# DSXiangLi/ChineseNER

Hardware: NVIDIA H100
Metric: sentences/sec bert_bilstm_crf MSRA L=128 (higher is better)
Workload: dtype bf16

## Files before the change

chinesener_b200/_lib.py:

```python
import ctypes
import os

import torch

_HERE = os.path.dirname(os.path.abspath(__file__))
LIB_PATH = os.path.join(_HERE, "libner_b200.so")

_c = ctypes
_vp, _i = _c.c_void_p, _c.c_int

SIGNATURES = {
    "ner_strerror": (_c.c_char_p, [_i]),
    "ner_abi_version": (_i, []),
    "ner_build_info": (_c.c_char_p, []),
    "ner_crf_viterbi": (_i, [_vp, _vp, _vp, _vp, _vp, _i, _i, _i, _vp]),
    "ner_crf_viterbi_plan": (_i, [_i, _i, _i, _i, _i]),
    "ner_crf_loglik_fwd": (_i, [_vp, _vp, _vp, _vp, _vp, _vp, _vp, _i, _i, _i, _i, _vp]),
    "ner_crf_loglik_bwd": (_i, [_vp, _vp, _vp, _vp, _vp, _vp, _vp, _c.c_float, _vp, _vp, _i, _i, _i, _vp]),
    "ner_gemm_bf16": (_i, [_vp, _vp, _vp, _vp, _vp, _i, _i, _i, _i, _i, _vp]),
    "ner_pack_weight_bf16": (_i, [_vp, _vp, _i, _i, _vp]),
    "ner_cast_bf16": (_i, [_vp, _vp, _c.c_size_t, _vp]),
    "ner_dense_small_n": (_i, [_vp, _i, _vp, _vp, _vp, _i, _i, _i, _vp, _vp]),
    "ner_seq_pack_plan": (_i, [_vp, _vp, _vp, _i, _i, _vp]),
    "ner_bert_embed_ln": (_i, [_vp] * 9 + [_i] * 6 + [_c.c_float, _vp, _i, _vp]),
    "ner_layernorm": (_i, [_vp, _i] + [_vp] * 5 + [_i, _i, _c.c_float, _vp]),
    "ner_layernorm_dropout": (_i, [_vp, _i] + [_vp] * 5 + [_i, _i, _c.c_float, _c.c_float, _c.c_uint64, _vp]),
    "ner_bert_attention": (_i, [_vp, _vp, _vp, _i, _i, _i, _i, _c.c_float, _c.c_float, _vp, _i, _c.c_float, _c.c_uint64, _vp]),
    "ner_bilstm_recurrence": (_i, [_vp] * 5 + [_i, _i, _i, _i, _c.c_float, _vp, _vp, _vp, _vp, _c.c_float, _c.c_uint64, _vp]),
    "ner_bilstm_recurrence_bwd": (_i, [_vp] * 7 + [_i, _i, _i, _i, _c.c_float, _c.c_uint64, _vp]),
    "ner_bigru_recurrence": (_i, [_vp] * 5 + [_i, _i, _i, _i, _i] + [_vp] * 4 + [_c.c_float, _c.c_uint64, _vp]),
    "ner_bigru_recurrence_bwd": (_i, [_vp] * 7 + [_i, _i, _i, _i, _c.c_float, _c.c_uint64, _vp]),
    "ner_transpose_cast_bf16": (_i, [_vp, _vp, _i, _i, _i, _i, _vp]),
    "ner_colsum_add": (_i, [_vp, _vp, _i, _i, _i, _c.c_float, _vp]),
    "ner_dense_small_n_bwd": (_i, [_vp] * 6 + [_i, _i, _i, _vp]),
    "ner_dropout": (_i, [_vp, _vp, _c.c_size_t, _c.c_float, _c.c_uint64, _vp]),
    "ner_relu_bwd_f32": (_i, [_vp, _vp, _vp, _c.c_size_t, _vp]),
    "ner_relu_f32": (_i, [_vp, _vp, _c.c_size_t, _vp]),
    "ner_reduce_max_time": (_i, [_vp, _vp, _i, _i, _i, _vp]),
    "ner_reduce_max_time_bwd": (_i, [_vp, _vp, _vp, _vp, _i, _i, _i, _c.c_float, _vp]),
    "ner_softmax_xent": (_i, [_vp, _vp, _vp, _vp, _i, _i, _c.c_float, _vp]),
    "ner_attention_f32_bwd": (_i, [_vp, _i, _vp, _i, _vp, _i, _vp, _vp, _vp, _vp, _c.c_float, _vp, _i, _vp, _i, _vp, _i, _vp, _i,
                                   _vp, _vp, _i, _i, _i, _i, _vp]),
    "ner_dropout_bf16": (_i, [_vp, _vp, _c.c_size_t, _c.c_float, _c.c_uint64, _vp]),
    "ner_sumsq_add": (_i, [_vp, _c.c_size_t, _vp, _vp, _vp]),
    "ner_sumsq_scratch_floats": (_c.c_size_t, []),
    "ner_token_xent": (_i, [_vp] * 6 + [_c.c_float, _vp, _i, _i, _i, _vp]),
    "ner_token_xent_scratch_floats": (_c.c_size_t, []),
    "ner_token_dice": (_i, [_vp] * 6 + [_c.c_float] * 3 + [_vp, _i, _i, _i, _vp]),
    "ner_mrc_pairs": (_i, [_vp] * 6 + [_i] * 6 + [_vp] * 7),
    "ner_mrc_merge": (_i, [_vp] * 3 + [_i] * 6 + [_vp, _vp]),
    "ner_mrc_span_targets": (_i, [_vp, _vp, _i, _i, _vp, _vp, _vp, _vp]),
    "ner_mrc_span_match_fwd_workspace_bytes": (_c.c_size_t, [_i, _i]),
    "ner_mrc_span_match_fwd": (_i, [_vp, _i] + [_vp] * 5 + [_i] * 3 + [_c.c_float, _c.c_uint64] + [_vp] * 3
                               + [_c.c_size_t, _vp]),
    "ner_mrc_span_match_bwd_workspace_bytes": (_c.c_size_t, [_i, _i]),
    "ner_mrc_span_match_bwd": (_i, [_vp, _i] + [_vp] * 5 + [_i] * 3 + [_c.c_float, _c.c_float, _c.c_uint64] + [_vp] * 5
                               + [_c.c_size_t, _vp]),
    "ner_mrc_span_decode_workspace_bytes": (_c.c_size_t, [_i, _i]),
    "ner_mrc_span_decode": (_i, [_vp] * 3 + [_i] + [_vp] * 5 + [_i] * 8 + [_vp] * 5 + [_c.c_size_t, _vp]),
    "ner_gp_targets": (_i, [_vp] * 3 + [_i] * 3 + [_vp, _vp]),
    "ner_gp_rope": (_i, [_vp, _i, _vp] + [_i] * 3 + [_vp] * 3),
    "ner_gp_rope_bwd": (_i, [_vp, _vp] + [_i] * 3 + [_vp, _i, _vp]),
    "ner_gp_loss_workspace_bytes": (_c.c_size_t, [_i] * 3),
    "ner_gp_loss_fwd": (_i, [_vp] * 5 + [_i] * 3 + [_vp] * 3 + [_c.c_size_t, _vp]),
    "ner_gp_loss_bwd": (_i, [_vp] * 5 + [_i] * 3 + [_c.c_float, _vp, _vp]),
    "ner_gp_decode_workspace_bytes": (_c.c_size_t, [_i] * 3),
    "ner_gp_decode": (_i, [_vp] * 5 + [_i] * 7 + [_vp] * 5 + [_c.c_size_t, _vp]),
    "ner_window_plan": (_i, [_vp] * 3 + [_i] * 5 + [_vp] * 6),
    "ner_layernorm_bwd": (_i, [_vp, _i] + [_vp] * 7 + [_i, _i, _c.c_float, _vp]),
    "ner_layernorm_dropout_bwd": (_i, [_vp, _i] + [_vp] * 7 + [_i, _i, _c.c_float, _c.c_float, _c.c_uint64, _vp]),
    "ner_layernorm_dropout_bwd_bias": (_i, [_vp, _i] + [_vp] * 8 + [_i, _i, _c.c_float, _c.c_float, _c.c_uint64, _vp]),
    "ner_transpose_bf16": (_i, [_vp, _vp, _i, _i, _i, _vp]),
    "ner_colsum_bf16_add": (_i, [_vp, _vp, _i, _i, _vp]),
    "ner_gelu_bf16": (_i, [_vp, _vp, _c.c_size_t, _i, _vp]),
    "ner_gelu_f32": (_i, [_vp, _vp, _c.c_size_t, _i, _vp]),
    "ner_gelu_bwd_bf16": (_i, [_vp, _vp, _vp, _c.c_size_t, _i, _vp]),
    "ner_gelu_bwd_bias_bf16": (_i, [_vp, _vp, _vp, _vp, _i, _i, _i, _vp]),
    "ner_bert_embed_bwd": (_i, [_vp] * 6 + [_i] * 5 + [_vp]),
    "ner_bert_attention_bwd": (_i, [_vp] * 5 + [_i] * 4 + [_c.c_float, _c.c_float, _c.c_float, _c.c_uint64, _vp]),
    "ner_bert_attention_bwd_packed": (_i, [_vp] * 5 + [_i] * 4 + [_c.c_float, _c.c_float, _c.c_uint64, _vp]),
    "ner_gather_rows": (_i, [_vp, _vp, _vp, _i, _i, _vp]),
# ... 148 lines not shown
```

chinesener_b200/csrc/bilstm.cu:

```cuda
#include <cooperative_groups.h>
#include <stdlib.h>

#include "common.cuh"
#include "dsmem.cuh"

namespace cg = cooperative_groups;

namespace {

__device__ __forceinline__ float sigmoidf_(float x) { return __fdividef(1.f, 1.f + __expf(-x)); }

template <int ACT>
__device__ __forceinline__ float actf(float x) {
  if (ACT == 1) return fmaxf(x, 0.f);
  return 1.f - __fdividef(2.f, 1.f + __expf(2.f * x));
}

template <int R, int ACT, int H4REG>
__global__ void __launch_bounds__(H4REG > 0 ? 256 : 512, 1) bilstm_rec_kernel(const float* __restrict__ xproj, const float* __restrict__ wh_fw,
                                  const float* __restrict__ wh_bw, const int32_t* __restrict__ seq_len,
                                  float* __restrict__ out, int B, int L, int H, int C, float forget_bias,
                                  const int32_t* __restrict__ cu_seqlens, float* __restrict__ gates_out,
                                  float* __restrict__ cstate_out, float* __restrict__ hstate_out, float keep_prob,
                                  uint32_t seed_lo, uint32_t seed_hi) {
  cg::cluster_group cluster = cg::this_cluster();
  const int rank = (int)cluster.block_rank();
  const int HU = H / C;
  const int NC = 4 * HU;
  const int H4 = H / 4;
  const int ngroups = (B + R - 1) / R;
  const int cid = blockIdx.x / C;
  const int dir = cid / ngroups;
  const int b0 = (cid % ngroups) * R;
  const int tid = threadIdx.x;

  extern __shared__ __align__(16) float smem[];
  constexpr bool WREG = H4REG > 0;
  float4* Ws4 = reinterpret_cast<float4*>(smem);
  float* hbuf = smem + (WREG ? 0 : (size_t)H * NC);
  int* s_len = reinterpret_cast<int*>(hbuf + 2 * R * H);
  uint64_t* hbar = reinterpret_cast<uint64_t*>(s_len + 8);

  const float* wh = dir == 0 ? wh_fw : wh_bw;
  float4 wreg[WREG ? H4REG : 1];
  if constexpr (WREG) {
    if (tid < NC) {
      const int g0 = tid & 3, u0 = tid >> 2;
      const size_t gc = (size_t)g0 * H + rank * HU + u0;
#pragma unroll
      for (int k4 = 0; k4 < H4REG; ++k4) {
        wreg[k4].x = wh[(size_t)(4 * k4 + 0) * 4 * H + gc];
        wreg[k4].y = wh[(size_t)(4 * k4 + 1) * 4 * H + gc];
        wreg[k4].z = wh[(size_t)(4 * k4 + 2) * 4 * H + gc];
        wreg[k4].w = wh[(size_t)(4 * k4 + 3) * 4 * H + gc];
      }
    }
  } else {
    for (int idx = tid; idx < H4 * NC; idx += blockDim.x) {
      const int k4 = idx / NC, col = idx - k4 * NC;
      const int g = col & 3, u = col >> 2;
      const size_t gc = (size_t)g * H + rank * HU + u;
      float4 w;
      w.x = wh[(size_t)(4 * k4 + 0) * 4 * H + gc];
      w.y = wh[(size_t)(4 * k4 + 1) * 4 * H + gc];
      w.z = wh[(size_t)(4 * k4 + 2) * 4 * H + gc];
      w.w = wh[(size_t)(4 * k4 + 3) * 4 * H + gc];
      Ws4[idx] = w;
    }
  }
  for (int idx = tid; idx < 2 * R * H; idx += blockDim.x) hbuf[idx] = 0.f;
  if (tid < R) s_len[tid] = (b0 + tid < B) ? min(max(seq_len[b0 + tid], 0), L) : 0;
  if (tid == 0) {
    mbar_init_(&hbar[0], 1);
    mbar_init_(&hbar[1], 1);
    asm volatile("fence.mbarrier_init.release.cluster;" ::: "memory");
  }
  __syncthreads();
  int maxlen = 0;
#pragma unroll
  for (int r = 0; r < R; ++r) maxlen = max(maxlen, s_len[r]);
  cluster.sync();

  const bool col_ok = tid < NC;
  const int g = tid & 3, u = tid >> 2;
  const int ug = rank * HU + u;
  const size_t xcol = (size_t)dir * 4 * H + (size_t)g * H + ug;
  constexpr int RC = (R + 3) / 4;
  float c_state[RC];
#pragma unroll
  for (int rr = 0; rr < RC; ++rr) c_state[rr] = 0.f;

  size_t xrow0[R];
#pragma unroll
  for (int r = 0; r < R; ++r)
    xrow0[r] = (b0 + r < B) ? (cu_seqlens ? (size_t)cu_seqlens[b0 + r] : (size_t)(b0 + r) * L) : 0;
  float xp[R];
#pragma unroll
  for (int r = 0; r < R; ++r) {
    xp[r] = 0.f;
    const int len = s_len[r];
    if (col_ok && 0 < len) {
      const int pos = dir == 0 ? 0 : len - 1;
      xp[r] = xproj[(xrow0[r] + pos) * 8 * H + xcol];
    }
  }
  const uint32_t thr = nerdev::keep_threshold(keep_prob);
  const float inv_keep = 1.f / keep_prob;

  const uint32_t h_bytes = (uint32_t)(R * H * 4);
  for (int s = 0; s < maxlen; ++s) {
    const float* hcur = hbuf + (s & 1) * R * H;
    float* hnxt = hbuf + ((s + 1) & 1) * R * H;
    if (C > 1) {
      if (tid == 0) mbar_arrive_expect_tx_(&hbar[(s + 1) & 1], h_bytes);
      if (s > 0) mbar_wait_(&hbar[s & 1], (uint32_t)((s - 1) >> 1) & 1u);
    }
    nerdev::f32x2 pa[R], pb[R];
#pragma unroll
    for (int r = 0; r < R; ++r) {
      pa[r] = nerdev::pk2(xp[r], 0.f);
      pb[r] = nerdev::pk2(0.f, 0.f);
    }
    if (col_ok) {
#pragma unroll
      for (int r = 0; r < R; ++r) {
        const int len = s_len[r];
        xp[r] = 0.f;
        if (s + 1 < len) {
          const int pos = dir == 0 ? s + 1 : len - 2 - s;
          xp[r] = xproj[(xrow0[r] + pos) * 8 * H + xcol];
        }
      }
      const float4* hc4 = reinterpret_cast<const float4*>(hcur);
      if constexpr (WREG) {
#pragma unroll
        for (int k4 = 0; k4 < H4REG; ++k4) {
          const float4 w = wreg[k4];
#pragma unroll
          for (int r = 0; r < R; ++r) {
            const float4 hv = hc4[r * H4 + k4];
            pa[r] = nerdev::fma2(nerdev::pk2(w.x, w.y), nerdev::pk2(hv.x, hv.y), pa[r]);
            pb[r] = nerdev::fma2(nerdev::pk2(w.z, w.w), nerdev::pk2(hv.z, hv.w), pb[r]);
          }
        }
      } else {
#pragma unroll 4
        for (int k4 = 0; k4 < H4; ++k4) {
          const float4 w = Ws4[k4 * NC + tid];
#pragma unroll
          for (int r = 0; r < R; ++r) {
            const float4 hv = hc4[r * H4 + k4];
            pa[r] = nerdev::fma2(nerdev::pk2(w.x, w.y), nerdev::pk2(hv.x, hv.y), pa[r]);
            pb[r] = nerdev::fma2(nerdev::pk2(w.z, w.w), nerdev::pk2(hv.z, hv.w), pb[r]);
          }
        }
      }
    }
    float zi[RC], zj[RC], zf[RC], zo[RC];
#pragma unroll
    for (int rr = 0; rr < RC; ++rr) zi[rr] = zj[rr] = zf[rr] = zo[rr] = 0.f;
    const int qb = (tid & 31) & ~3;
#pragma unroll
    for (int r = 0; r < R; ++r) {
      float z0, z1, z2, z3;
      nerdev::upk2(pa[r], z0, z1);
      nerdev::upk2(pb[r], z2, z3);
      const float z = (z0 + z1) + (z2 + z3);
      const float a0 = __shfl_sync(0xffffffffu, z, qb + 0);
      const float a1 = __shfl_sync(0xffffffffu, z, qb + 1);
      const float a2 = __shfl_sync(0xffffffffu, z, qb + 2);
      const float a3 = __shfl_sync(0xffffffffu, z, qb + 3);
      if (g == (r & 3)) {
        zi[r >> 2] = a0;
        zj[r >> 2] = a1;
        zf[r >> 2] = a2;
        zo[r >> 2] = a3;
      }
    }
#pragma unroll
    for (int rr = 0; rr < RC; ++rr) {
      const int r = g + 4 * rr;
      const bool cell_ok = col_ok && r < R;
      float i_s = 0.f, j_a = 0.f, f_s = 0.f, o_s = 0.f, h_out = 0.f, h_state = 0.f;
      const int len = cell_ok ? s_len[r] : 0;
      const int b = b0 + r;
      const bool live = cell_ok && s < len;
      const int pos = dir == 0 ? s : len - 1 - s;
      if (live) {
        i_s = sigmoidf_(zi[rr]);
        j_a = actf<ACT>(zj[rr]);
        f_s = sigmoidf_(zf[rr] + forget_bias);
        o_s = sigmoidf_(zo[rr]);
        c_state[rr] = f_s * c_state[rr] + i_s * j_a;
        const float h_raw = o_s * actf<ACT>(c_state[rr]);
        h_out = h_raw;
        h_state = h_raw;
        if (keep_prob < 1.f) {
          const uint32_t e = (uint32_t)(((size_t)b * L + pos) * 2 * H + (size_t)dir * H + ug);
          h_out = nerdev::hash3(seed_lo, seed_hi, e) < thr ? h_raw * inv_keep : 0.f;
          h_state = nerdev::hash3(seed_lo ^ 0x5bd1e995u, seed_hi, e) < thr ? h_raw * inv_keep : 0.f;
        }
      }
      if (cell_ok) {
        if (C > 1) {
          const uint32_t la = nerdev::smem_u32(hnxt + r * H + ug), lb = nerdev::smem_u32(&hbar[(s + 1) & 1]);
          for (int dst = 0; dst < C; ++dst) st_async_f32(mapa_u32(la, (uint32_t)dst), h_state, mapa_u32(lb, (uint32_t)dst));
        } else {
          hnxt[r * H + ug] = h_state;
        }
      }
      if (live) {
        out[((size_t)b * L + pos) * 2 * H + (size_t)dir * H + ug] = h_out;
        if (hstate_out != nullptr) hstate_out[((size_t)b * L + pos) * 2 * H + (size_t)dir * H + ug] = h_state;
        if (gates_out != nullptr) {
          const size_t gi = ((size_t)b * L + pos) * 8 * H + (size_t)dir * 4 * H;
          gates_out[gi + 0 * H + ug] = i_s;
          gates_out[gi + 1 * H + ug] = j_a;
          gates_out[gi + 2 * H + ug] = f_s;
          gates_out[gi + 3 * H + ug] = o_s;
          cstate_out[((size_t)b * L + pos) * 2 * H + (size_t)dir * H + ug] = c_state[rr];
        }
      } else if (cell_ok && b < B) {
        out[((size_t)b * L + s) * 2 * H + (size_t)dir * H + ug] = 0.f;
      }
    }
    if (C == 1) __syncthreads();
  }
  if (C > 1) cluster.sync();

  for (int idx = tid; idx < R * HU; idx += blockDim.x) {
    const int r = idx / HU, uu = idx - r * HU;
    const int b = b0 + r;
    if (b < B)
      for (int s = maxlen; s < L; ++s) out[((size_t)b * L + s) * 2 * H + (size_t)dir * H + rank * HU + uu] = 0.f;
  }
}

int pick_cluster(int H) {
  for (int C = 1; C <= 8; C *= 2) {
    if (H % C != 0) continue;
    const size_t bytes = (size_t)H * 4 * (H / C) * 4;
    if (bytes <= 190 * 1024 && 4 * (H / C) <= 512) return C;
  }
  return 0;
}

template <int R, int ACT, int H4REG>
int launch_rec(const float* xproj, const float* wh_fw, const float* wh_bw, const int32_t* seq_len, float* out, int B,
               int L, int H, int C, float forget_bias, const int32_t* cu_seqlens, float* gates_out, float* cstate_out,
               float* hstate_out, float keep_prob, uint64_t seed, cudaStream_t st) {
  const int HU = H / C, NC = 4 * HU;
  const size_t smem = ((H4REG > 0 ? 0 : (size_t)H * NC) + 2 * R * H + 32) * 4;
  auto kern = bilstm_rec_kernel<R, ACT, H4REG>;
  cudaError_t e = cudaFuncSetAttribute(kern, cudaFuncAttributeMaxDynamicSharedMemorySize, (int)smem);
  if (e != cudaSuccess) return NER_ERR_CUDA_BASE - (int)e;
  const int ngroups = (B + R - 1) / R;
  cudaLaunchConfig_t cfg{};
  cfg.gridDim = dim3((unsigned)(2 * ngroups * C));
  cfg.blockDim = dim3((unsigned)((NC + 31) / 32 * 32));
  cfg.dynamicSmemBytes = smem;
  cfg.stream = st;
  cudaLaunchAttribute attr[1];
  attr[0].id = cudaLaunchAttributeClusterDimension;
  attr[0].val.clusterDim.x = (unsigned)C;
  attr[0].val.clusterDim.y = 1;
  attr[0].val.clusterDim.z = 1;
  cfg.attrs = attr;
  cfg.numAttrs = 1;
  e = cudaLaunchKernelEx(&cfg, kern, xproj, wh_fw, wh_bw, seq_len, out, B, L, H, C, forget_bias, cu_seqlens, gates_out,
                         cstate_out, hstate_out, keep_prob, (uint32_t)seed, (uint32_t)(seed >> 32));
  if (e != cudaSuccess) return NER_ERR_CUDA_BASE - (int)e;
  return ner_launch_status();
}

}

extern "C" int ner_bilstm_recurrence(const float* xproj, const float* wh_fw, const float* wh_bw,
                                     const int32_t* seq_len, float* out, int B, int L, int H, int activation,
                                     float forget_bias, const int32_t* cu_seqlens, float* gates_out,
                                     float* cstate_out, float* hstate_out, float keep_prob, uint64_t seed,
                                     ner_stream_t stream) {
  if (B < 0 || L < 1 || H < 1) return NER_ERR_INVALID_ARG;
  if (B == 0) return NER_OK;
  if (!xproj || !wh_fw || !wh_bw || !seq_len || !out) return NER_ERR_INVALID_ARG;
  if ((gates_out == nullptr) != (cstate_out == nullptr)) return NER_ERR_INVALID_ARG;
  if (!(keep_prob > 0.f) || keep_prob > 1.f) return NER_ERR_INVALID_ARG;
  if (activation != 0 && activation != 1) return NER_ERR_INVALID_ARG;
  if (H % 4 != 0) return NER_ERR_UNSUPPORTED;
  const int C = pick_cluster(H);
  if (C == 0) return NER_ERR_UNSUPPORTED;
  cudaStream_t st = static_cast<cudaStream_t>(stream);
  int R = 1;
  if ((long)2 * B * C > ner_num_sms()) R = 2;
  if ((long)2 * ((B + 1) / 2) * C > 2 * ner_num_sms()) R = 4;
  if (H == 128 && (long)2 * ((B + 3) / 4) * C > ner_num_sms()) R = 8;
  if (const char* e = getenv("NER_BILSTM_ROWS")) {
    const int v = atoi(e);
    if (v == 1 || v == 2 || v == 4 || (v == 8 && H == 128)) R = v;
  }
#define GO(RR, HR)                                                                                          \
  return activation == 1 ? launch_rec<RR, 1, HR>(xproj, wh_fw, wh_bw, seq_len, out, B, L, H, C, forget_bias, cu_seqlens, gates_out, cstate_out, hstate_out, keep_prob, seed, st) \
                         : launch_rec<RR, 0, HR>(xproj, wh_fw, wh_bw, seq_len, out, B, L, H, C, forget_bias, cu_seqlens, gates_out, cstate_out, hstate_out, keep_prob, seed, st)
  if (H == 128 && 4 * (H / C) <= 256) {
    if (R == 8) GO(8, 32);
    if (R == 4) GO(4, 32);
    if (R == 2) GO(2, 32);
    GO(1, 32);
  }
  if (R >= 4) GO(4, 0);
  if (R == 2) GO(2, 0);
  GO(1, 0);
#undef GO
}
```

chinesener_b200/csrc/predict_step.cu:

```cuda
#include "common.cuh"

namespace {
inline size_t al256(size_t x) { return (x + 255) & ~(size_t)255; }
}

extern "C" size_t ner_bert_bilstm_crf_predict_workspace_bytes(const ner_bert_config* cfg, int B, int L, int rows,
                                                              int lstm_hidden, int num_tags) {
  if (!cfg || B < 0 || L < 1 || rows < 0) return 0;
  const size_t H = (size_t)cfg->hidden_size, R = (size_t)rows, Hl = (size_t)lstm_hidden;
  return al256((size_t)(B + 1) * 4)
         + al256((size_t)B * L * 4)
         + al256(R * H * 4) + al256(R * H * 2)
         + al256(R * 8 * Hl * 4)
         + al256((size_t)B * L * 2 * Hl * 4)
         + al256((size_t)B * L * num_tags * 4)
         + ner_bert_encoder_workspace_bytes(cfg, rows);
}

extern "C" int ner_bert_bilstm_crf_predict(const ner_bert_config* cfg, const float* word_emb, const float* type_emb,
                                           const float* pos_emb, const float* emb_ln_gamma, const float* emb_ln_beta,
                                           const ner_bert_layer_weights* layers, const void* lstm_wx_bf16,
                                           const float* lstm_bias, const float* lstm_wh_fw, const float* lstm_wh_bw,
                                           int lstm_hidden, int lstm_activation, const float* logits_w,
                                           const float* logits_b, const float* trans, int num_tags, const int32_t* ids,
                                           const int32_t* mask, const int32_t* seg, const int32_t* seq_len, int B, int L,
                                           int n_packed, int32_t* pred_ids, void* workspace, size_t workspace_bytes,
                                           ner_stream_t stream) {
  if (!cfg || !layers || !lstm_wx_bf16 || !lstm_bias || !lstm_wh_fw || !lstm_wh_bw || !logits_w || !logits_b || !trans ||
      !ids || !mask || !seq_len || !pred_ids || !workspace)
    return NER_ERR_INVALID_ARG;
  if (B < 0 || L < 1 || n_packed < 0 || n_packed > B * L) return NER_ERR_INVALID_ARG;
  if (B == 0) return NER_OK;
  const int H = cfg->hidden_size, Hl = lstm_hidden, K = num_tags;
  if (H % 8 != 0) return NER_ERR_UNSUPPORTED;
  if (workspace_bytes < ner_bert_bilstm_crf_predict_workspace_bytes(cfg, B, L, n_packed, Hl, K)) return NER_ERR_WORKSPACE;
  cudaStream_t st = static_cast<cudaStream_t>(stream);
  uint8_t* p = static_cast<uint8_t*>(workspace);
  int32_t* cu = reinterpret_cast<int32_t*>(p);       p += al256((size_t)(B + 1) * 4);
  int32_t* tok_src = reinterpret_cast<int32_t*>(p);  p += al256((size_t)B * L * 4);
  float* x32 = reinterpret_cast<float*>(p);          p += al256((size_t)n_packed * H * 4);
  void* x16 = p;                                     p += al256((size_t)n_packed * H * 2);
  float* xproj = reinterpret_cast<float*>(p);        p += al256((size_t)n_packed * 8 * Hl * 4);
  float* lstm_out = reinterpret_cast<float*>(p);     p += al256((size_t)B * L * 2 * Hl * 4);
  float* logits = reinterpret_cast<float*>(p);       p += al256((size_t)B * L * K * 4);
  void* enc_ws = p;
  const size_t enc_bytes = ner_bert_encoder_workspace_bytes(cfg, n_packed);

  int rc = ner_seq_pack_plan(mask, cu, tok_src, B, L, stream);
  if (rc != NER_OK) return rc;
  if (n_packed == 0) {
    if (cudaMemsetAsync(pred_ids, 0, (size_t)B * L * 4, st) != cudaSuccess) return NER_ERR_CUDA_BASE - (int)cudaGetLastError();
    return NER_OK;
  }
  rc = ner_bert_encoder_fwd(cfg, word_emb, type_emb, pos_emb, emb_ln_gamma, emb_ln_beta, layers, ids, mask, seg, B, L, cu,
                            tok_src, n_packed, x32, x16, enc_ws, enc_bytes, stream);
  if (rc != NER_OK) return rc;
  rc = ner_gemm_bf16(x16, lstm_wx_bf16, lstm_bias, nullptr, xproj, n_packed, 8 * Hl, H, NER_EPI_F32, cfg->gemm_tile, stream);
  if (rc != NER_OK) return rc;
  rc = ner_bilstm_recurrence(xproj, lstm_wh_fw, lstm_wh_bw, seq_len, lstm_out, B, L, Hl, lstm_activation, 1.0f, cu, nullptr,
                             nullptr, nullptr, 1.0f, 0, stream);
  if (rc != NER_OK) return rc;
  rc = ner_dense_small_n(lstm_out, 0, logits_w, logits_b, logits, B * L, 2 * Hl, K, nullptr, stream);
  if (rc != NER_OK) return rc;
  return ner_crf_viterbi(logits, seq_len, trans, pred_ids, nullptr, B, L, K, stream);
}
```

chinesener_b200/fastpath.py:

```python
import ctypes

import torch

from . import _lib, bert as _bert, ops
from .tools import layer as _layer

_ws = {}


def _workspace(nbytes, device):
    key = (device.index, _lib.stream())
    ws = _ws.get(key)
    if ws is None or ws.numel() < nbytes:
        ws = _ws[key] = torch.empty((nbytes,), dtype=torch.uint8, device=device)
    return ws


def bert_bilstm_crf_predict(est, dev):
    store, params = est.store, est.params
    mask = dev['mask']
    total = getattr(mask, "total_tokens", None)
    if total is None or not _layer.PACK_SEQUENCES or _bert.PER_KERNEL or params.get('bert_precision', _layer.BERT_PRECISION) != 'bf16':
        return None
    if params.get('cell_type', 'lstm').lower() != 'lstm' or params.get('cell_size', 1) != 1:
        return None
    if dev['token_ids'].shape[1] > est.document_window()[0]:
        return None
    Hl, K = params['hidden_units_list'][0], params['label_size']
    v = store.vars
    lscope = "bilstm_layer/bidirectional_rnn"
    need = ("logits/kernel", "logits/bias", "crf_layer/transitions", f"{lscope}/fw/multi_rnn_cell/cell_0/lstm_cell/kernel",
            "bert/embeddings/word_embeddings")
    if any(n not in v for n in need):
        return None
    cfg = _bert.load_bert_config(params['pretrain_dir'])
    H = cfg["hidden_size"]
    c, arr, _ = _bert._c_tables(store, cfg, "bert", "tanh")
    c.gemm_tile = ops.DEFAULT_TILE
    pk = _layer._rnn_pack(store, {d: _layer._rnn_names(lscope, d, "lstm", 0) for d in ("fw", "bw")}, H, False)
    if pk["Dp"] != H:
        return None
    ids, seg, m32, sl = ops._i32(dev['token_ids']), ops._i32(dev['segment_ids']), ops._i32(mask), ops._i32(dev['seq_len'])
    B, L = ids.shape
    lib = _lib.lib()
    nbytes = lib.ner_bert_bilstm_crf_predict_workspace_bytes(ctypes.byref(c), B, L, int(total), Hl, K)
    ws = _workspace(nbytes, ids.device)
    pred = torch.empty((B, L), dtype=torch.int32, device=ids.device)
    emb = [v[f"bert/embeddings/{n}"] for n in ("word_embeddings", "token_type_embeddings", "position_embeddings",
                                               "LayerNorm/gamma", "LayerNorm/beta")]
    _lib.check(lib.ner_bert_bilstm_crf_predict(
        ctypes.byref(c), *[t.data_ptr() for t in emb], arr, pk["wx"].data_ptr(), pk["bias"].data_ptr(), pk["wh_fw"].data_ptr(),
        pk["wh_bw"].data_ptr(), Hl, 1 if params['rnn_activation'] == 'relu' else 0, v["logits/kernel"].data_ptr(),
        v["logits/bias"].data_ptr(), v["crf_layer/transitions"].data_ptr(), K, ids.data_ptr(), m32.data_ptr(), seg.data_ptr(),
        sl.data_ptr(), B, L, int(total), pred.data_ptr(), ws.data_ptr(), ws.numel(), _lib.stream()))
    _lib.LAUNCHES += 5 + 7 * cfg["num_hidden_layers"]
    return pred


FUSED_PREDICT = {"bert_bilstm_crf": bert_bilstm_crf_predict}
```

chinesener_b200/ops.py:

```python
import torch

from . import _lib
from ._lib import NerB200Error, check, lib, ptr, require_cuda, stream

EPI_F32, EPI_BF16, EPI_GELU_TANH_BF16, EPI_GELU_ERF_BF16, EPI_RELU_BF16, EPI_RES_F32, EPI_RES_RELU_F32 = range(7)
EPI_DIAG_DISCARD = 99
EPI_GELU_TANH_E4M3, EPI_GELU_ERF_E4M3 = 7, 8
E4M3 = torch.float8_e4m3fn
TILE_2CTA_128, TILE_2CTA_256 = 1128, 1256
TILE_SK_128, TILE_SK_256 = 2128, 2256
TILE_AUTO_THROUGHPUT = 3000
DEFAULT_TILE = 0


def _i32(t):
    return t if t.dtype == torch.int32 else t.to(torch.int32)


def crf_viterbi(logits, seq_len, trans, return_score=False):
    require_cuda(logits, seq_len, trans)
    assert logits.dtype == torch.float32 and trans.dtype == torch.float32
    B, L, K = logits.shape
    assert trans.shape == (K, K)
    seq_len = _i32(seq_len)
# ... 134 lines not shown
def layernorm(y, gamma, beta, residual=None, eps=1e-12, want_f32=True, want_bf16=True, keep_prob=1.0, seed=0):
    require_cuda(y, gamma, beta, residual)
    assert y.dtype in (torch.float32, torch.bfloat16)
    M, H = y.shape
    of = torch.empty((M, H), dtype=torch.float32, device=y.device) if want_f32 else None
    ob = torch.empty((M, H), dtype=torch.bfloat16, device=y.device) if want_bf16 else None
    check(lib().ner_layernorm_dropout(ptr(y), 1 if y.dtype == torch.bfloat16 else 0, ptr(residual), ptr(gamma), ptr(beta),
                                      ptr(of), ptr(ob), M, H, eps, float(keep_prob), int(seed) & 0xFFFFFFFFFFFFFFFF, stream()))
    return of, ob


def bert_embed_ln_e4m3(word_emb, type_emb, pos_emb, gamma, beta, ids, seg, eps=1e-12, tok_src=None, n_packed=0):
    require_cuda(word_emb, type_emb, pos_emb, gamma, beta, ids, seg, tok_src)
    B, L = ids.shape
    V, H = word_emb.shape
    ids = _i32(ids)
    seg = None if seg is None else _i32(seg)
    rows = n_packed if tok_src is not None else B * L
    of = torch.empty((rows, H), dtype=torch.float32, device=ids.device)
    oq = torch.empty((rows, H), dtype=E4M3, device=ids.device)
    osc = torch.empty((rows, H // 128), dtype=torch.float32, device=ids.device)
    check(lib().ner_bert_embed_ln_e4m3(ptr(word_emb), ptr(type_emb), ptr(pos_emb), ptr(gamma), ptr(beta), ptr(ids), ptr(seg),
                                       ptr(of), None, ptr(oq), ptr(osc), B, L, H, V, type_emb.shape[0], pos_emb.shape[0], eps,
                                       ptr(tok_src), n_packed, stream()))
    return of, oq, osc


def layernorm_e4m3(y, gamma, beta, residual=None, eps=1e-12):
    require_cuda(y, gamma, beta, residual)
    assert y.dtype in (torch.float32, torch.bfloat16)
    M, H = y.shape
    of = torch.empty((M, H), dtype=torch.float32, device=y.device)
    oq = torch.empty((M, H), dtype=E4M3, device=y.device)
    osc = torch.empty((M, H // 128), dtype=torch.float32, device=y.device)
    check(lib().ner_layernorm_e4m3(ptr(y), 1 if y.dtype == torch.bfloat16 else 0, ptr(residual), ptr(gamma), ptr(beta),
                                   ptr(of), None, ptr(oq), ptr(osc), M, H, eps, stream()))
    return of, oq, osc


def bert_attention(qkv, mask, B, L, num_heads, head_dim=64, scale=None, mask_add=-10000.0, cu_seqlens=None, keep_prob=1.0,
                   seed=0):
    require_cuda(qkv, mask, cu_seqlens)
    assert qkv.dtype == torch.bfloat16 and qkv.shape[1] == 3 * num_heads * head_dim
    assert cu_seqlens is not None or qkv.shape[0] == B * L
    mask = None if mask is None else _i32(mask)
    ctx = torch.empty((qkv.shape[0], num_heads * head_dim), dtype=torch.bfloat16, device=qkv.device)
    if scale is None:
        scale = 1.0 / (head_dim ** 0.5)
    check(lib().ner_bert_attention(ptr(qkv), ptr(mask), ptr(ctx), B, L, num_heads, head_dim, scale, mask_add,
                                   ptr(cu_seqlens), int(qkv.shape[0]), float(keep_prob), int(seed) & 0xFFFFFFFFFFFFFFFF, stream()))
    return ctx


def bilstm_recurrence(xproj, wh_fw, wh_bw, seq_len, B, L, H, activation="tanh", forget_bias=1.0, cu_seqlens=None,
                      save_for_backward=False, keep_prob=1.0, seed=0):
    require_cuda(xproj, wh_fw, wh_bw, seq_len, cu_seqlens)
    assert xproj.dtype == torch.float32 and xproj.shape[1] == 8 * H
    assert cu_seqlens is not None or xproj.shape[0] == B * L
    assert wh_fw.shape == (H, 4 * H) and wh_bw.shape == (H, 4 * H)
    act = {"tanh": 0, "relu": 1}[activation]
    out = torch.empty((B, L, 2 * H), dtype=torch.float32, device=xproj.device)
    gates = cst = hst = None
    if save_for_backward:
        assert cu_seqlens is None, "training runs on the padded layout"
        gates = torch.zeros((B * L, 8 * H), dtype=torch.float32, device=xproj.device)
        cst = torch.zeros((B, L, 2 * H), dtype=torch.float32, device=xproj.device)
        hst = torch.zeros((B, L, 2 * H), dtype=torch.float32, device=xproj.device)
    check(lib().ner_bilstm_recurrence(ptr(xproj), ptr(wh_fw), ptr(wh_bw), ptr(_i32(seq_len)), ptr(out), B, L, H, act,
                                      forget_bias, ptr(cu_seqlens), ptr(gates), ptr(cst), ptr(hst), float(keep_prob),
                                      int(seed) & 0xFFFFFFFFFFFFFFFF, stream()))
    return (out, gates, cst, hst) if save_for_backward else out


def bilstm_recurrence_bwd(d_out, gates, cstate, wh_fw, wh_bw, seq_len, B, L, H, activation="tanh", keep_prob=1.0, seed=0):
    require_cuda(d_out, gates, cstate, wh_fw, wh_bw, seq_len)
    assert d_out.shape == (B, L, 2 * H) and d_out.dtype == torch.float32
    act = {"tanh": 0, "relu": 1}[activation]
    d_xproj = torch.empty((B * L, 8 * H), dtype=torch.float32, device=d_out.device)
    check(lib().ner_bilstm_recurrence_bwd(ptr(d_out), ptr(gates), ptr(cstate), ptr(wh_fw), ptr(wh_bw), ptr(_i32(seq_len)),
                                          ptr(d_xproj), B, L, H, act, float(keep_prob), int(seed) & 0xFFFFFFFFFFFFFFFF,
                                          stream()))
    return d_xproj


def bigru_recurrence(xproj, wh_fw, wh_bw, seq_len, B, L, H, activation="tanh", cu_seqlens=None, save_for_backward=False,
                     keep_prob=1.0, seed=0):
    require_cuda(xproj, wh_fw, wh_bw, seq_len, cu_seqlens)
    assert xproj.dtype == torch.float32 and xproj.shape[1] >= 6 * H
    assert cu_seqlens is not None or xproj.shape[0] == B * L
    assert wh_fw.shape == (H, 3 * H) and wh_bw.shape == (H, 3 * H)
    act = {"tanh": 0, "relu": 1}[activation]
    out = torch.empty((B, L, 2 * H), dtype=torch.float32, device=xproj.device)
    gates = hst = rh = None
    if save_for_backward:
        assert cu_seqlens is None, "training runs on the padded layout"
        gates = torch.zeros((B * L, 6 * H), dtype=torch.float32, device=xproj.device)
        hst = torch.zeros((B, L, 2 * H), dtype=torch.float32, device=xproj.device)
        rh = torch.zeros((B, L, 2 * H), dtype=torch.float32, device=xproj.device)
    check(lib().ner_bigru_recurrence(ptr(xproj), ptr(wh_fw), ptr(wh_bw), ptr(_i32(seq_len)), ptr(out), B, L, H, xproj.shape[1],
                                     act, ptr(cu_seqlens), ptr(gates), ptr(hst), ptr(rh), float(keep_prob),
                                     int(seed) & 0xFFFFFFFFFFFFFFFF, stream()))
    return (out, gates, hst, rh) if save_for_backward else out


def bigru_recurrence_bwd(d_out, gates, hstate, wh_fw, wh_bw, seq_len, B, L, H, activation="tanh", keep_prob=1.0, seed=0):
    require_cuda(d_out, gates, hstate, wh_fw, wh_bw, seq_len)
    assert d_out.shape == (B, L, 2 * H) and d_out.dtype == torch.float32
    assert gates.shape == (B * L, 6 * H) and hstate.shape == (B, L, 2 * H)
    act = {"tanh": 0, "relu": 1}[activation]
    d_xproj = torch.empty((B * L, 6 * H), dtype=torch.float32, device=d_out.device)
    check(lib().ner_bigru_recurrence_bwd(ptr(d_out), ptr(gates), ptr(hstate), ptr(wh_fw), ptr(wh_bw), ptr(_i32(seq_len)),
                                         ptr(d_xproj), B, L, H, act, float(keep_prob), int(seed) & 0xFFFFFFFFFFFFFFFF,
                                         stream()))
    return d_xproj


def lattice_recurrence(xproj, wproj, lat_len, wrec_fw, wrec_bw, wac_fw, wac_bw, seq_len, B, L, H, Kw,
                       save_for_backward=False):
    require_cuda(xproj, wproj, lat_len, wrec_fw, wrec_bw, wac_fw, wac_bw, seq_len)
    assert xproj.dtype == torch.float32 and xproj.shape == (B * L, 8 * H)
    assert wproj.dtype == torch.float32 and wproj.shape == (B * L * Kw, 6 * H)
    assert lat_len.dtype == torch.int32 and lat_len.numel() == B * L * Kw
    assert wrec_fw.shape == (H, 6 * H) and wrec_bw.shape == (H, 6 * H) and wac_fw.shape == (H, H) and wac_bw.shape == (H, H)
# ... 759 lines not shown
```

include/ner_b200.h:

```cpp
#ifndef NER_B200_H_
#define NER_B200_H_

#include <stddef.h>
#include <stdint.h>

#ifdef __cplusplus
extern "C" {
#endif

#define NER_OK 0
#define NER_ERR_INVALID_ARG (-1)
#define NER_ERR_UNSUPPORTED (-2)
#define NER_ERR_WORKSPACE (-3)
#define NER_ERR_NO_DRIVER (-4)
#define NER_ERR_CUDA_BASE (-1000)

typedef void* ner_stream_t;

const char* ner_strerror(int status);
int ner_abi_version(void);
const char* ner_build_info(void);


int ner_crf_viterbi(const float* logits, const int32_t* seq_len, const float* trans,
// ... 174 lines not shown
                               const float* pos_emb, const float* emb_ln_gamma, const float* emb_ln_beta,
                               const ner_bert_layer_weights* layers, const int32_t* ids,
                               const int32_t* mask, const int32_t* seg, int B, int L,
                               float hidden_keep, float attn_keep, uint64_t seed, float* out_f32,
                               void* out_bf16, void* saved, size_t saved_bytes, ner_stream_t stream);
int ner_bert_encoder_train_bwd(const ner_bert_config* cfg, const float* emb_ln_gamma,
                               const ner_bert_layer_weights* layers, const ner_bert_layer_grads* grads,
                               float* d_word_emb, float* d_type_emb, float* d_pos_emb,
                               float* d_emb_ln_gamma, float* d_emb_ln_beta, const int32_t* ids,
                               const int32_t* mask, const int32_t* seg, int B, int L,
                               float hidden_keep, float attn_keep, uint64_t seed, const float* d_out,
                               const void* saved, size_t saved_bytes, void* scratch,
                               size_t scratch_bytes, ner_stream_t stream);
size_t ner_bert_train_packed_saved_bytes(const ner_bert_config* cfg, int n_packed);
size_t ner_bert_train_packed_scratch_bytes(const ner_bert_config* cfg, int n_packed, int padded_rows);
int ner_bert_encoder_train_fwd_packed(const ner_bert_config* cfg, const float* word_emb, const float* type_emb,
                                      const float* pos_emb, const float* emb_ln_gamma, const float* emb_ln_beta,
                                      const ner_bert_layer_weights* layers, const int32_t* ids, const int32_t* seg,
                                      int B, int L, const int32_t* cu_seqlens, const int32_t* tok_src, int n_packed,
                                      float hidden_keep, float attn_keep, uint64_t seed, float* out_f32,
                                      void* out_bf16, void* saved, size_t saved_bytes, ner_stream_t stream);
int ner_bert_encoder_train_bwd_packed(const ner_bert_config* cfg, const float* emb_ln_gamma,
                                      const ner_bert_layer_weights* layers, const ner_bert_layer_grads* grads,
                                      float* d_word_emb, float* d_type_emb, float* d_pos_emb,
                                      float* d_emb_ln_gamma, float* d_emb_ln_beta, const int32_t* ids,
                                      const int32_t* seg, int B, int L, const int32_t* cu_seqlens,
                                      const int32_t* tok_src, int n_packed, float hidden_keep, float attn_keep,
                                      uint64_t seed, const float* d_out, const void* saved, size_t saved_bytes,
                                      void* scratch, size_t scratch_bytes, ner_stream_t stream);
int ner_gather_rows(const void* src, const int32_t* idx, void* dst, int n, int row_bytes, ner_stream_t stream);
int ner_scatter_rows(const void* src, const int32_t* idx, void* dst, int n, int row_bytes, ner_stream_t stream);
int ner_bert_embed_sum(const float* word_emb, const float* type_emb, const float* pos_emb,
                       const int32_t* ids, const int32_t* seg, float* out, int B, int L, int H,
                       int vocab, int n_type, int max_pos, ner_stream_t stream);

size_t ner_bert_bilstm_crf_predict_workspace_bytes(const ner_bert_config* cfg, int B, int L, int rows,
                                                   int lstm_hidden, int num_tags);
int ner_bert_bilstm_crf_predict(const ner_bert_config* cfg, const float* word_emb, const float* type_emb,
                                const float* pos_emb, const float* emb_ln_gamma, const float* emb_ln_beta,
                                const ner_bert_layer_weights* layers, const void* lstm_wx_bf16,
                                const float* lstm_bias, const float* lstm_wh_fw, const float* lstm_wh_bw,
                                int lstm_hidden, int lstm_activation, const float* logits_w,
                                const float* logits_b, const float* trans, int num_tags,
                                const int32_t* ids, const int32_t* mask, const int32_t* seg,
                                const int32_t* seq_len, int B, int L, int n_packed, int32_t* pred_ids,
                                void* workspace, size_t workspace_bytes, ner_stream_t stream);


int ner_bilstm_recurrence(const float* xproj, const float* wh_fw, const float* wh_bw,
                          const int32_t* seq_len, float* out, int B, int L, int H,
                          int activation, float forget_bias, const int32_t* cu_seqlens,
                          float* gates_out, float* cstate_out, float* hstate_out, float keep_prob,
                          uint64_t seed, ner_stream_t stream);

int ner_bilstm_recurrence_bwd(const float* d_out, const float* gates, const float* cstate,
                              const float* wh_fw, const float* wh_bw, const int32_t* seq_len,
                              float* d_xproj, int B, int L, int H, int activation, float keep_prob,
                              uint64_t seed, ner_stream_t stream);


int ner_bigru_recurrence(const float* xproj, const float* wh_fw, const float* wh_bw, const int32_t* seq_len,
                         float* out, int B, int L, int H, int ld_xproj, int activation,
                         const int32_t* cu_seqlens, float* gates_out, float* hstate_out, float* rh_out, float keep_prob, uint64_t seed,
                         ner_stream_t stream);

int ner_bigru_recurrence_bwd(const float* d_out, const float* gates, const float* hstate, const float* wh_fw,
                             const float* wh_bw, const int32_t* seq_len, float* d_xproj, int B, int L, int H,
                             int activation, float keep_prob, uint64_t seed, ner_stream_t stream);


int ner_softlexicon_pool_fwd(const float* table, const int32_t* ids, const float* weights,
                             float* out, int n_tok, int G, int S, int E, int V, int ld_out,
                             ner_stream_t stream);
int ner_softlexicon_pool_bwd(float* d_table, const int32_t* ids, const float* weights,
                             const float* d_out, int n_tok, int G, int S, int E, int V,
                             ner_stream_t stream);


int ner_multihot_embed_fwd(const float* table, const float* weights, float* out, int n_tok, int V, int E,
                           int ld_out, ner_stream_t stream);
size_t ner_small_table_grad_scratch_floats(int V, int E);
int ner_small_table_grad(float* d_table, const int32_t* ids, const float* weights, const float* d_out, int n_tok,
                         int V, int E, int ld_dout, float* scratch, ner_stream_t stream);


int ner_transpose_cast_bf16(const float* src, void* dst_bf16, int M, int N, int Mp, int ld_src,
                            ner_stream_t stream);
int ner_colsum_add(const float* x, float* out, int M, int N, int ld, float scale,
                   ner_stream_t stream);
int ner_dense_small_n_bwd(const float* x, const float* W, const float* dy, float* dW, float* db,
                          float* dx, int M, int F, int N, ner_stream_t stream);
int ner_dropout(const float* x, float* y, size_t n, float keep_prob, uint64_t seed,
                ner_stream_t stream);
int ner_dropout_bf16(const void* x_bf16, void* y_bf16, size_t n, float keep_prob, uint64_t seed,
                     ner_stream_t stream);
int ner_relu_f32(const float* x, float* y, size_t n, ner_stream_t stream);
int ner_relu_bwd_f32(const float* act, const float* dact, float* dpre, size_t n, ner_stream_t stream);
int ner_reduce_max_time(const float* x, float* y, int B, int L, int C, ner_stream_t stream);
int ner_reduce_max_time_bwd(const float* x, const float* y, const float* dy, float* dx, int B, int L, int C,
                            float scale, ner_stream_t stream);
int ner_softmax_xent(const float* logits, const int32_t* labels, float* loss, float* dlogits, int B, int N,
                     float scale, ner_stream_t stream);
size_t ner_token_xent_scratch_floats(void);
int ner_token_xent(const float* logits, const int32_t* labels, const int32_t* seq_len, int32_t* pred_ids, float* loss,
                   float* d_logits, float d_loss, float* scratch, int B, int L, int K, ner_stream_t stream);
int ner_token_dice(const float* logits, const int32_t* labels, const int32_t* seq_len, int32_t* pred_ids, float* loss,
// ... 129 lines not shown
```

Before: 49580.

## Sort BiLSTM rows by sequence length and fix rows-per-cluster in throughput mode

Adds a single-block counting-sort kernel that orders batch rows by descending sequence length. The BiLSTM recurrence kernel now takes a row_order indirection, so each cluster handles rows of similar length and its loop bound (the group's longest row) wastes fewer steps on padding. In throughput tile mode it also fixes R=4 rows per cluster for the register-weight path instead of using the SM-count heuristic. This costs one extra small launch and a gather indirection, and it only takes effect when gemm_tile is the throughput policy.

Result: faster. 50620, median of 6 (+2.1%).

```diff
diff --git a/chinesener_b200/_lib.py b/chinesener_b200/_lib.py
--- a/chinesener_b200/_lib.py
+++ b/chinesener_b200/_lib.py
@@ -27,6 +27,9 @@
     "ner_layernorm_dropout": (_i, [_vp, _i] + [_vp] * 5 + [_i, _i, _c.c_float, _c.c_float, _c.c_uint64, _vp]),
     "ner_bert_attention": (_i, [_vp, _vp, _vp, _i, _i, _i, _i, _c.c_float, _c.c_float, _vp, _i, _c.c_float, _c.c_uint64, _vp]),
     "ner_bilstm_recurrence": (_i, [_vp] * 5 + [_i, _i, _i, _i, _c.c_float, _vp, _vp, _vp, _vp, _c.c_float, _c.c_uint64, _vp]),
+    "ner_bilstm_recurrence_ex": (_i, [_vp] * 5 + [_i, _i, _i, _i, _c.c_float, _vp, _vp, _i, _vp, _vp, _vp, _c.c_float, _c.c_uint64,
+                                          _vp]),
+    "ner_seq_len_order": (_i, [_vp, _vp, _i, _i, _vp]),
     "ner_bilstm_recurrence_bwd": (_i, [_vp] * 7 + [_i, _i, _i, _i, _c.c_float, _c.c_uint64, _vp]),
     "ner_bigru_recurrence": (_i, [_vp] * 5 + [_i, _i, _i, _i, _i] + [_vp] * 4 + [_c.c_float, _c.c_uint64, _vp]),
     "ner_bigru_recurrence_bwd": (_i, [_vp] * 7 + [_i, _i, _i, _i, _c.c_float, _c.c_uint64, _vp]),
diff --git a/chinesener_b200/csrc/bilstm.cu b/chinesener_b200/csrc/bilstm.cu
--- a/chinesener_b200/csrc/bilstm.cu
+++ b/chinesener_b200/csrc/bilstm.cu
@@ -20,9 +20,9 @@
 __global__ void __launch_bounds__(H4REG > 0 ? 256 : 512, 1) bilstm_rec_kernel(const float* __restrict__ xproj, const float* __restrict__ wh_fw,
                                   const float* __restrict__ wh_bw, const int32_t* __restrict__ seq_len,
                                   float* __restrict__ out, int B, int L, int H, int C, float forget_bias,
-                                  const int32_t* __restrict__ cu_seqlens, float* __restrict__ gates_out,
-                                  float* __restrict__ cstate_out, float* __restrict__ hstate_out, float keep_prob,
-                                  uint32_t seed_lo, uint32_t seed_hi) {
+                                  const int32_t* __restrict__ cu_seqlens, const int32_t* __restrict__ row_order,
+                                  float* __restrict__ gates_out, float* __restrict__ cstate_out,
+                                  float* __restrict__ hstate_out, float keep_prob, uint32_t seed_lo, uint32_t seed_hi) {
   cg::cluster_group cluster = cg::this_cluster();
   const int rank = (int)cluster.block_rank();
   const int HU = H / C;
@@ -39,7 +39,8 @@
   float4* Ws4 = reinterpret_cast<float4*>(smem);
   float* hbuf = smem + (WREG ? 0 : (size_t)H * NC);
   int* s_len = reinterpret_cast<int*>(hbuf + 2 * R * H);
-  uint64_t* hbar = reinterpret_cast<uint64_t*>(s_len + 8);
+  int* s_row = s_len + 8;
+  uint64_t* hbar = reinterpret_cast<uint64_t*>(s_len + 16);
 
   const float* wh = dir == 0 ? wh_fw : wh_bw;
   float4 wreg[WREG ? H4REG : 1];
@@ -69,7 +70,11 @@
     }
   }
   for (int idx = tid; idx < 2 * R * H; idx += blockDim.x) hbuf[idx] = 0.f;
-  if (tid < R) s_len[tid] = (b0 + tid < B) ? min(max(seq_len[b0 + tid], 0), L) : 0;
+  if (tid < R) {
+    const int b = b0 + tid >= B ? B : row_order ? row_order[b0 + tid] : b0 + tid;
+    s_row[tid] = b;
+    s_len[tid] = b < B ? min(max(seq_len[b], 0), L) : 0;
+  }
   if (tid == 0) {
     mbar_init_(&hbar[0], 1);
     mbar_init_(&hbar[1], 1);
@@ -92,8 +97,10 @@
 
   size_t xrow0[R];
 #pragma unroll
-  for (int r = 0; r < R; ++r)
-    xrow0[r] = (b0 + r < B) ? (cu_seqlens ? (size_t)cu_seqlens[b0 + r] : (size_t)(b0 + r) * L) : 0;
+  for (int r = 0; r < R; ++r) {
+    const int b = s_row[r];
+    xrow0[r] = b < B ? (cu_seqlens ? (size_t)cu_seqlens[b] : (size_t)b * L) : 0;
+  }
   float xp[R];
 #pragma unroll
   for (int r = 0; r < R; ++r) {
@@ -183,7 +190,7 @@
       const bool cell_ok = col_ok && r < R;
       float i_s = 0.f, j_a = 0.f, f_s = 0.f, o_s = 0.f, h_out = 0.f, h_state = 0.f;
       const int len = cell_ok ? s_len[r] : 0;
-      const int b = b0 + r;
+      const int b = cell_ok ? s_row[r] : B;
       const bool live = cell_ok && s < len;
       const int pos = dir == 0 ? s : len - 1 - s;
       if (live) {
@@ -230,9 +237,63 @@
 
   for (int idx = tid; idx < R * HU; idx += blockDim.x) {
     const int r = idx / HU, uu = idx - r * HU;
-    const int b = b0 + r;
+    const int b = s_row[r];
     if (b < B)
       for (int s = maxlen; s < L; ++s) out[((size_t)b * L + s) * 2 * H + (size_t)dir * H + rank * HU + uu] = 0.f;
+  }
+}
+
+__global__ void __launch_bounds__(1024) seq_len_order_kernel(const int32_t* __restrict__ seq_len,
+                                                             int32_t* __restrict__ row_order, int B, int L) {
+  extern __shared__ int s_key[];
+  __shared__ int s_warp[32];
+  const int nk = L + 1, tid = threadIdx.x, lane = tid & 31, warp = tid >> 5;
+  for (int k = tid; k < nk; k += blockDim.x) s_key[k] = 0;
+  __syncthreads();
+  for (int b = tid; b < B; b += blockDim.x) atomicAdd(&s_key[L - min(max(seq_len[b], 0), L)], 1);
+  __syncthreads();
+  const int per = (nk + blockDim.x - 1) / blockDim.x, k0 = min(tid * per, nk), k1 = min(k0 + per, nk);
+  int sum = 0;
+  for (int k = k0; k < k1; ++k) sum += s_key[k];
+  int incl = sum;
+#pragma unroll
+  for (int o = 1; o < 32; o <<= 1) {
+    const int v = __shfl_up_sync(0xffffffffu, incl, o);
+    if (lane >= o) incl += v;
+  }
+  if (lane == 31) s_warp[warp] = incl;
+  __syncthreads();
+  if (warp == 0) {
+    int w = lane < (int)(blockDim.x >> 5) ? s_warp[lane] : 0;
+#pragma unroll
+    for (int o = 1; o < 32; o <<= 1) {
+      const int v = __shfl_up_sync(0xffffffffu, w, o);
+      if (lane >= o) w += v;
+    }
+    s_warp[lane] = w;
+  }
+  __syncthreads();
+  int run = incl - sum + (warp > 0 ? s_warp[warp - 1] : 0);
+  for (int k = k0; k < k1; ++k) {
+    const int c = s_key[k];
+    s_key[k] = run;
+    run += c;
+  }
+  __syncthreads();
+  if (warp == 0) {
+    for (int base = 0; base < B; base += 32) {
+      const int b = base + lane;
+      const int key = b < B ? L - min(max(seq_len[b], 0), L) : -1;
+      const unsigned peers = __match_any_sync(0xffffffffu, key);
+      const int before = __popc(peers & ((1u << lane) - 1u));
+      const int slot = b < B ? s_key[key] + before : 0;
+      __syncwarp();
+      if (b < B) {
+        row_order[slot] = b;
+        if (before == __popc(peers) - 1) s_key[key] = slot + 1;
+      }
+      __syncwarp();
+    }
   }
 }
 
@@ -247,8 +308,8 @@
 
 template <int R, int ACT, int H4REG>
 int launch_rec(const float* xproj, const float* wh_fw, const float* wh_bw, const int32_t* seq_len, float* out, int B,
-               int L, int H, int C, float forget_bias, const int32_t* cu_seqlens, float* gates_out, float* cstate_out,
-               float* hstate_out, float keep_prob, uint64_t seed, cudaStream_t st) {
+               int L, int H, int C, float forget_bias, const int32_t* cu_seqlens, const int32_t* row_order,
+               float* gates_out, float* cstate_out, float* hstate_out, float keep_prob, uint64_t seed, cudaStream_t st) {
   const int HU = H / C, NC = 4 * HU;
   const size_t smem = ((H4REG > 0 ? 0 : (size_t)H * NC) + 2 * R * H + 32) * 4;
   auto kern = bilstm_rec_kernel<R, ACT, H4REG>;
@@ -267,12 +328,26 @@
   attr[0].val.clusterDim.z = 1;
   cfg.attrs = attr;
   cfg.numAttrs = 1;
-  e = cudaLaunchKernelEx(&cfg, kern, xproj, wh_fw, wh_bw, seq_len, out, B, L, H, C, forget_bias, cu_seqlens, gates_out,
-                         cstate_out, hstate_out, keep_prob, (uint32_t)seed, (uint32_t)(seed >> 32));
+  e = cudaLaunchKernelEx(&cfg, kern, xproj, wh_fw, wh_bw, seq_len, out, B, L, H, C, forget_bias, cu_seqlens, row_order,
+                         gates_out, cstate_out, hstate_out, keep_prob, (uint32_t)seed, (uint32_t)(seed >> 32));
   if (e != cudaSuccess) return NER_ERR_CUDA_BASE - (int)e;
   return ner_launch_status();
 }
 
+}
+
+extern "C" int ner_seq_len_order(const int32_t* seq_len, int32_t* row_order, int B, int L, ner_stream_t stream) {
+  if (B < 0 || L < 1) return NER_ERR_INVALID_ARG;
+  if (B == 0) return NER_OK;
+  if (!seq_len || !row_order) return NER_ERR_INVALID_ARG;
+  const size_t smem = (size_t)(L + 1) * 4;
+  if (smem > 200 * 1024) return NER_ERR_UNSUPPORTED;
+  if (smem > 48 * 1024) {
+    cudaError_t e = cudaFuncSetAttribute(seq_len_order_kernel, cudaFuncAttributeMaxDynamicSharedMemorySize, (int)smem);
+    if (e != cudaSuccess) return NER_ERR_CUDA_BASE - (int)e;
+  }
+  seq_len_order_kernel<<<1, 1024, smem, static_cast<cudaStream_t>(stream)>>>(seq_len, row_order, B, L);
+  return ner_launch_status();
 }
 
 extern "C" int ner_bilstm_recurrence(const float* xproj, const float* wh_fw, const float* wh_bw,
@@ -280,6 +355,15 @@
                                      float forget_bias, const int32_t* cu_seqlens, float* gates_out,
                                      float* cstate_out, float* hstate_out, float keep_prob, uint64_t seed,
                                      ner_stream_t stream) {
+  return ner_bilstm_recurrence_ex(xproj, wh_fw, wh_bw, seq_len, out, B, L, H, activation, forget_bias, cu_seqlens,
+                                  nullptr, 0, gates_out, cstate_out, hstate_out, keep_prob, seed, stream);
+}
+
+extern "C" int ner_bilstm_recurrence_ex(const float* xproj, const float* wh_fw, const float* wh_bw,
+                                        const int32_t* seq_len, float* out, int B, int L, int H, int activation,
+                                        float forget_bias, const int32_t* cu_seqlens, const int32_t* row_order,
+                                        int tile_policy, float* gates_out, float* cstate_out, float* hstate_out,
+                                        float keep_prob, uint64_t seed, ner_stream_t stream) {
   if (B < 0 || L < 1 || H < 1) return NER_ERR_INVALID_ARG;
   if (B == 0) return NER_OK;
   if (!xproj || !wh_fw || !wh_bw || !seq_len || !out) return NER_ERR_INVALID_ARG;
@@ -289,19 +373,25 @@
   if (H % 4 != 0) return NER_ERR_UNSUPPORTED;
   const int C = pick_cluster(H);
   if (C == 0) return NER_ERR_UNSUPPORTED;
+  if (tile_policy != 0 && tile_policy != NER_TILE_AUTO_THROUGHPUT) return NER_ERR_INVALID_ARG;
   cudaStream_t st = static_cast<cudaStream_t>(stream);
+  const bool wreg = H == 128 && 4 * (H / C) <= 256;
   int R = 1;
-  if ((long)2 * B * C > ner_num_sms()) R = 2;
-  if ((long)2 * ((B + 1) / 2) * C > 2 * ner_num_sms()) R = 4;
-  if (H == 128 && (long)2 * ((B + 3) / 4) * C > ner_num_sms()) R = 8;
+  if (tile_policy == NER_TILE_AUTO_THROUGHPUT && wreg) {
+    R = 4;
+  } else {
+    if ((long)2 * B * C > ner_num_sms()) R = 2;
+    if ((long)2 * ((B + 1) / 2) * C > 2 * ner_num_sms()) R = 4;
+    if (H == 128 && (long)2 * ((B + 3) / 4) * C > ner_num_sms()) R = 8;
+  }
   if (const char* e = getenv("NER_BILSTM_ROWS")) {
     const int v = atoi(e);
     if (v == 1 || v == 2 || v == 4 || (v == 8 && H == 128)) R = v;
   }
 #define GO(RR, HR)                                                                                          \
-  return activation == 1 ? launch_rec<RR, 1, HR>(xproj, wh_fw, wh_bw, seq_len, out, B, L, H, C, forget_bias, cu_seqlens, gates_out, cstate_out, hstate_out, keep_prob, seed, st) \
-                         : launch_rec<RR, 0, HR>(xproj, wh_fw, wh_bw, seq_len, out, B, L, H, C, forget_bias, cu_seqlens, gates_out, cstate_out, hstate_out, keep_prob, seed, st)
-  if (H == 128 && 4 * (H / C) <= 256) {
+  return activation == 1 ? launch_rec<RR, 1, HR>(xproj, wh_fw, wh_bw, seq_len, out, B, L, H, C, forget_bias, cu_seqlens, row_order, gates_out, cstate_out, hstate_out, keep_prob, seed, st) \
+                         : launch_rec<RR, 0, HR>(xproj, wh_fw, wh_bw, seq_len, out, B, L, H, C, forget_bias, cu_seqlens, row_order, gates_out, cstate_out, hstate_out, keep_prob, seed, st)
+  if (wreg) {
     if (R == 8) GO(8, 32);
     if (R == 4) GO(4, 32);
     if (R == 2) GO(2, 32);
diff --git a/chinesener_b200/csrc/predict_step.cu b/chinesener_b200/csrc/predict_step.cu
--- a/chinesener_b200/csrc/predict_step.cu
+++ b/chinesener_b200/csrc/predict_step.cu
@@ -9,6 +9,7 @@
   if (!cfg || B < 0 || L < 1 || rows < 0) return 0;
   const size_t H = (size_t)cfg->hidden_size, R = (size_t)rows, Hl = (size_t)lstm_hidden;
   return al256((size_t)(B + 1) * 4)
+         + al256((size_t)B * 4)
          + al256((size_t)B * L * 4)
          + al256(R * H * 4) + al256(R * H * 2)
          + al256(R * 8 * Hl * 4)
@@ -37,6 +38,7 @@
   cudaStream_t st = static_cast<cudaStream_t>(stream);
   uint8_t* p = static_cast<uint8_t*>(workspace);
   int32_t* cu = reinterpret_cast<int32_t*>(p);       p += al256((size_t)(B + 1) * 4);
+  int32_t* order = reinterpret_cast<int32_t*>(p);    p += al256((size_t)B * 4);
   int32_t* tok_src = reinterpret_cast<int32_t*>(p);  p += al256((size_t)B * L * 4);
   float* x32 = reinterpret_cast<float*>(p);          p += al256((size_t)n_packed * H * 4);
   void* x16 = p;                                     p += al256((size_t)n_packed * H * 2);
@@ -57,8 +59,11 @@
   if (rc != NER_OK) return rc;
   rc = ner_gemm_bf16(x16, lstm_wx_bf16, lstm_bias, nullptr, xproj, n_packed, 8 * Hl, H, NER_EPI_F32, cfg->gemm_tile, stream);
   if (rc != NER_OK) return rc;
-  rc = ner_bilstm_recurrence(xproj, lstm_wh_fw, lstm_wh_bw, seq_len, lstm_out, B, L, Hl, lstm_activation, 1.0f, cu, nullptr,
-                             nullptr, nullptr, 1.0f, 0, stream);
+  const bool thr = cfg->gemm_tile == NER_TILE_AUTO_THROUGHPUT;
+  if (thr && (rc = ner_seq_len_order(seq_len, order, B, L, stream)) != NER_OK) return rc;
+  rc = ner_bilstm_recurrence_ex(xproj, lstm_wh_fw, lstm_wh_bw, seq_len, lstm_out, B, L, Hl, lstm_activation, 1.0f, cu,
+                                thr ? order : nullptr, thr ? NER_TILE_AUTO_THROUGHPUT : 0, nullptr, nullptr, nullptr, 1.0f, 0,
+                                stream);
   if (rc != NER_OK) return rc;
   rc = ner_dense_small_n(lstm_out, 0, logits_w, logits_b, logits, B * L, 2 * Hl, K, nullptr, stream);
   if (rc != NER_OK) return rc;
diff --git a/chinesener_b200/fastpath.py b/chinesener_b200/fastpath.py
--- a/chinesener_b200/fastpath.py
+++ b/chinesener_b200/fastpath.py
@@ -53,7 +53,7 @@
         pk["wh_bw"].data_ptr(), Hl, 1 if params['rnn_activation'] == 'relu' else 0, v["logits/kernel"].data_ptr(),
         v["logits/bias"].data_ptr(), v["crf_layer/transitions"].data_ptr(), K, ids.data_ptr(), m32.data_ptr(), seg.data_ptr(),
         sl.data_ptr(), B, L, int(total), pred.data_ptr(), ws.data_ptr(), ws.numel(), _lib.stream()))
-    _lib.LAUNCHES += 5 + 7 * cfg["num_hidden_layers"]
+    _lib.LAUNCHES += 5 + 7 * cfg["num_hidden_layers"] + (c.gemm_tile == ops.TILE_AUTO_THROUGHPUT)
     return pred
 
 
diff --git a/chinesener_b200/ops.py b/chinesener_b200/ops.py
--- a/chinesener_b200/ops.py
+++ b/chinesener_b200/ops.py
@@ -210,9 +210,18 @@
     return ctx
 
 
+def seq_len_order(seq_len, L):
+    require_cuda(seq_len)
+    seq_len = _i32(seq_len)
+    order = torch.empty((seq_len.numel(),), dtype=torch.int32, device=seq_len.device)
+    check(lib().ner_seq_len_order(ptr(seq_len), ptr(order), seq_len.numel(), L, stream()))
+    return order
+
+
 def bilstm_recurrence(xproj, wh_fw, wh_bw, seq_len, B, L, H, activation="tanh", forget_bias=1.0, cu_seqlens=None,
-                      save_for_backward=False, keep_prob=1.0, seed=0):
-    require_cuda(xproj, wh_fw, wh_bw, seq_len, cu_seqlens)
+                      save_for_backward=False, keep_prob=1.0, seed=0, row_order=None, tile_policy=0):
+    require_cuda(xproj, wh_fw, wh_bw, seq_len, cu_seqlens, row_order)
+    assert row_order is None or (row_order.dtype == torch.int32 and row_order.numel() == B)
     assert xproj.dtype == torch.float32 and xproj.shape[1] == 8 * H
     assert cu_seqlens is not None or xproj.shape[0] == B * L
     assert wh_fw.shape == (H, 4 * H) and wh_bw.shape == (H, 4 * H)
@@ -224,9 +233,9 @@
         gates = torch.zeros((B * L, 8 * H), dtype=torch.float32, device=xproj.device)
         cst = torch.zeros((B, L, 2 * H), dtype=torch.float32, device=xproj.device)
         hst = torch.zeros((B, L, 2 * H), dtype=torch.float32, device=xproj.device)
-    check(lib().ner_bilstm_recurrence(ptr(xproj), ptr(wh_fw), ptr(wh_bw), ptr(_i32(seq_len)), ptr(out), B, L, H, act,
-                                      forget_bias, ptr(cu_seqlens), ptr(gates), ptr(cst), ptr(hst), float(keep_prob),
-                                      int(seed) & 0xFFFFFFFFFFFFFFFF, stream()))
+    check(lib().ner_bilstm_recurrence_ex(ptr(xproj), ptr(wh_fw), ptr(wh_bw), ptr(_i32(seq_len)), ptr(out), B, L, H, act,
+                                         forget_bias, ptr(cu_seqlens), ptr(row_order), tile_policy, ptr(gates), ptr(cst),
+                                         ptr(hst), float(keep_prob), int(seed) & 0xFFFFFFFFFFFFFFFF, stream()))
     return (out, gates, cst, hst) if save_for_backward else out
 
 
diff --git a/include/ner_b200.h b/include/ner_b200.h
--- a/include/ner_b200.h
+++ b/include/ner_b200.h
@@ -250,6 +250,13 @@
                           int activation, float forget_bias, const int32_t* cu_seqlens,
                           float* gates_out, float* cstate_out, float* hstate_out, float keep_prob,
                           uint64_t seed, ner_stream_t stream);
+int ner_bilstm_recurrence_ex(const float* xproj, const float* wh_fw, const float* wh_bw,
+                             const int32_t* seq_len, float* out, int B, int L, int H,
+                             int activation, float forget_bias, const int32_t* cu_seqlens,
+                             const int32_t* row_order, int tile_policy, float* gates_out,
+                             float* cstate_out, float* hstate_out, float keep_prob, uint64_t seed,
+                             ner_stream_t stream);
+int ner_seq_len_order(const int32_t* seq_len, int32_t* row_order, int B, int L, ner_stream_t stream);
 
 int ner_bilstm_recurrence_bwd(const float* d_out, const float* gates, const float* cstate,
                               const float* wh_fw, const float* wh_bw, const int32_t* seq_len,
```
